# suryanshkumar/online-joint-depthfusion-and-semantic

Hardware: AMD Instinct MI355X
Metric: frames/sec fused (320x240, 256^3 grid) (higher is better)
Workload: dtype f16x3; 1 GPU; BASELINE configs[1]: 320x240 depth into a 256^3 fp16 TSDF grid, FusionNet_v3, geometry-only, fast integrate, f16x3 arithmetic, one scene per GPU; grid=256, n_points=9, n_tail_points=7, volume_dtype=f16, parallelism=scene-sharded x1, cpu_affinity=not pinned

## Files before the change

### include/ojf.h

```cpp
#ifndef OJF_H
#define OJF_H

#include <stddef.h>
#include <stdint.h>

#ifdef __cplusplus
extern "C" {
#endif

typedef void *ojf_stream_t;

#define OJF_MODE_FAST 0
#define OJF_MODE_PARITY 1

#define OJF_ACT_NONE 0
#define OJF_ACT_RELU 1
#define OJF_ACT_LEAKY 2
#define OJF_ACT_TANH 3

#define OJF_ARITH_F32 0
#define OJF_ARITH_F16X3 1

const char *ojf_version(void);
const char *ojf_last_error(void);
// ... 32 lines not shown
typedef struct ojf_net ojf_net;
typedef struct ojf_conv_layer {
    int c_in, c_out, ksize, dilation;
    const float *weight_host;
    const float *bias_host;
} ojf_conv_layer;

int ojf_net_create(ojf_net **out, int version, int n_points, int growth, int use_semantics,
                   float output_scale, const ojf_conv_layer *layers_host, int n_layers, int h,
                   int w);
void ojf_net_destroy(ojf_net *net);
int ojf_net_layer_count(int version, int n_points, int growth, int use_semantics);
int ojf_net_prepare_input(ojf_net *net, const float *values_dev, const float *weights_dev, int rows_stride,
                          int in_layout, const float *depth_dev, const uint8_t *sem_ids_dev, int n_classes,
                          ojf_stream_t stream);
int ojf_net_forward(ojf_net *net, float *est_dev, int est_stride, ojf_stream_t stream);
int64_t ojf_net_macs_per_pixel(const ojf_net *net);
int ojf_net_launch_count(const ojf_net *net);
int ojf_net_side_streams(ojf_net *net, ojf_stream_t stream, ojf_stream_t out[3]);
int ojf_net_profile(ojf_net *net, float *est_dev, int est_stride, ojf_stream_t stream, char *names, int names_cap,
                    float *micros, int max_entries);
int ojf_net_plan(int version, int n_points, int growth, int use_semantics, int h, int w, int arithmetic, char *names,
                 int names_cap);
int ojf_net_set_arithmetic(int arithmetic);
int ojf_net_get_arithmetic(const ojf_net *net);
int ojf_net_check(ojf_stream_t stream);
int ojf_guard_status(ojf_stream_t stream, int *flag, int *skipped);
int ojf_guard_poll(void);
int ojf_streams_overlap(ojf_stream_t a, ojf_stream_t b);

int ojf_conv2d(const float *in_dev, int in_stride, int in_off, float *out_dev, int out_stride,
               int out_off, const ojf_conv_layer *layer_host, int act, int h, int w,
               ojf_stream_t stream);

#define OJF_SEG_ACT_ZERO_PAD 0x100
typedef struct ojf_segconv ojf_segconv;
int ojf_segconv_create(ojf_segconv **out, const float *weight_host, const float *scale_host, const float *bias_host,
                       int c_in, int c_out, int ksize, int stride, int dilation, int padding);
int ojf_segdeconv_create(ojf_segconv **out, const float *weight_host, const float *scale_host, const float *bias_host,
                         int c_in, int c_out, int stride);
void ojf_segconv_destroy(ojf_segconv *conv);
int ojf_segconv_set_dropout(ojf_segconv *conv, const unsigned long long *rng_state_dev, unsigned stream_id, int advance);
int ojf_segconv_forward(const ojf_segconv *conv, const float *in_dev, int in_stride, float *out_dev, int out_stride,
                        const float *res_dev, int res_stride, const float *mul_dev, int mul_stride, int act, int h,
                        int w, ojf_stream_t stream);
int ojf_segconv_forward_group(int n, const ojf_segconv *const *convs, const float *const *ins_dev, int in_stride,
                              float *const *outs_dev, int out_stride, const float *const *ress_dev, int res_stride,
                              const float *const *muls_dev, int mul_stride, int act, int h, int w, ojf_stream_t stream);
int ojf_segconv_forward_multi(int n, int batch, const ojf_segconv *const *convs, const float *const *ins_dev, const int *in_strides,
                              float *const *outs_dev, const int *out_strides, const float *const *ress_dev, const int *res_strides,
                              const float *const *muls_dev, const int *mul_strides, const int *acts, const int *hs, const int *ws,
                              ojf_stream_t stream);
int ojf_segconv_forward_batch(const ojf_segconv *conv, int batch, const float *in_dev, int in_stride, float *out_dev, int out_stride,
                              const float *res_dev, int res_stride, const float *mul_dev, int mul_stride, int act, int h,
                              int w, ojf_stream_t stream);
int ojf_segconv_forward_group_batch(int n, int batch, const ojf_segconv *const *convs, const float *const *ins_dev, int in_stride,
                                    float *const *outs_dev, int out_stride, const float *const *ress_dev, int res_stride,
                                    const float *const *muls_dev, int mul_stride, int act, int h, int w, ojf_stream_t stream);

size_t ojf_train_packed_floats(int c_out_phys, int c_in_phys, int ksize);
int ojf_train_pack(const float *w_dev, const float *bias_dev, int oc, int ic, int ksize, int group, int slot, int c_in_phys,
                   int c_out_phys, int transposed, float *packed_dev, float *bias_packed_dev, ojf_stream_t stream);
int ojf_train_conv(const float *in_dev, int in_g0, int c_in_phys, float *out_dev, int out_g0, int c_out_phys,
                   const float *packed_dev, const float *bias_packed_dev, int ksize, int dilation, int h, int w, ojf_stream_t stream);
int ojf_train_avgpool3(const float *in_dev, float *out_dev, int c_phys, int h, int w, ojf_stream_t stream);
size_t ojf_train_partial_doubles(int c_phys);
// ... 201 lines not shown
```

### online_joint_depthfusion_and_semantic_amd/_lib.py

```python
import ctypes
import os

import numpy as np

_HERE = os.path.dirname(os.path.abspath(__file__))
LIB_PATH = os.path.join(_HERE, 'libojf.so')
if os.environ.get('OJF_LIB_PATH'):
    LIB_PATH = os.environ['OJF_LIB_PATH']

MODE_FAST = 0
MODE_PARITY = 1
ACT_NONE, ACT_RELU, ACT_LEAKY, ACT_TANH = 0, 1, 2, 3
ARITH_F32, ARITH_F16X3 = 0, 1
ARITHMETIC = {'f32': ARITH_F32, 'f16x3': ARITH_F16X3}


class OjfError(RuntimeError):
    pass


class ConvLayer(ctypes.Structure):
    _fields_ = [('c_in', ctypes.c_int), ('c_out', ctypes.c_int), ('ksize', ctypes.c_int),
                ('dilation', ctypes.c_int), ('weight_host', ctypes.c_void_p),
                ('bias_host', ctypes.c_void_p)]
# ... 35 lines not shown

SIGNATURES = {
    'ojf_version': (_c.c_char_p, []),
    'ojf_last_error': (_c.c_char_p, []),
    'ojf_device_count': (_i, []),
    'ojf_extract': (_i, [_vp, _vp, _vp, _vp, _d, _vp, _vp, _i, _i, _i, _i, _i, _i, _f, _vp, _vp, _i, _i,
                         _vp, _vp, _vp, _vp, _vp]),
    'ojf_extract_to_net': (_i, [_vp, _vp, _vp, _vp, _d, _vp, _vp, _i, _i, _i, _i, _i, _i, _f, _vp, _vp]),
    'ojf_extract_many': (_i, [_i, _c.POINTER(ExtractJob), _i, _i, _i, _i, _i, _i, _f, _vp]),
    'ojf_integrate_many': (_i, [_i, _c.POINTER(IntegrateJob), _i, _i, _f, _i, _i, _i, _i, _i, _vp]),
    'ojf_integrate_workspace_bytes': (_sz, [_i, _i, _i, _i, _i, _i, _i]),
    'ojf_integrate_workspace_init': (_i, [_vp, _sz, _i, _i, _i, _i, _i, _i, _i, _vp]),
    'ojf_integrate': (_i, [_vp, _vp, _vp, _vp, _d, _vp, _i, _i, _i, _f, _vp, _vp, _vp, _vp, _vp, _vp,
                           _i, _i, _i, _i, _i, _i, _vp, _sz, _vp, _vp]),
    'ojf_integrate_masked': (_i, [_vp, _vp, _vp, _vp, _vp, _d, _vp, _i, _i, _i, _f, _vp, _vp, _vp, _vp, _vp, _vp,
                                  _i, _i, _i, _i, _i, _i, _vp, _sz, _vp, _vp]),
    'ojf_integrate_entries': (_i, [_vp, _vp, _vp, _vp, _vp, _c.c_int64, _vp, _vp, _vp, _vp, _i, _i, _i, _vp, _sz, _vp, _vp]),
    'ojf_net_create': (_i, [_c.POINTER(_vp), _i, _i, _i, _i, _f, _c.POINTER(ConvLayer), _i, _i, _i]),
    'ojf_net_destroy': (None, [_vp]),
    'ojf_net_layer_count': (_i, [_i, _i, _i, _i]),
    'ojf_net_prepare_input': (_i, [_vp, _vp, _vp, _i, _i, _vp, _vp, _i, _vp]),
    'ojf_net_forward': (_i, [_vp, _vp, _i, _vp]),
    'ojf_net_macs_per_pixel': (_c.c_int64, [_vp]),
    'ojf_net_launch_count': (_i, [_vp]),
    'ojf_net_side_streams': (_i, [_vp, _vp, _vp]),
    'ojf_net_profile': (_i, [_vp, _vp, _i, _vp, _c.c_char_p, _i, _c.POINTER(_f), _i]),
    'ojf_net_plan': (_i, [_i, _i, _i, _i, _i, _i, _i, _c.c_char_p, _i]),
    'ojf_net_set_arithmetic': (_i, [_i]),
    'ojf_net_get_arithmetic': (_i, [_vp]),
    'ojf_net_check': (_i, [_vp]),
    'ojf_guard_status': (_i, [_vp, _c.POINTER(_i), _c.POINTER(_i)]),
    'ojf_guard_poll': (_i, []),
    'ojf_streams_overlap': (_i, [_vp, _vp]),
    'ojf_conv2d': (_i, [_vp, _i, _i, _vp, _i, _i, _c.POINTER(ConvLayer), _i, _i, _i, _vp]),
    'ojf_volume_fill_f16': (_i, [_vp, _sz, _f, _vp]),
    'ojf_volume_fill_u8': (_i, [_vp, _sz, _c.c_uint8, _vp]),
    'ojf_volume_filter': (_i, [_vp, _vp, _sz, _f, _f, _vp]),
    'ojf_volume_median5_u8': (_i, [_vp, _vp, _i, _i, _i, _vp]),
    'ojf_volume_evaluate': (_i, [_vp, _vp, _vp, _sz, _vp, _vp]),
    'ojf_volume_confusion': (_i, [_vp, _vp, _vp, _sz, _i, _vp, _vp, _vp]),
    'ojf_segconv_create': (_i, [_c.POINTER(_vp), _vp, _vp, _vp, _i, _i, _i, _i, _i, _i]),
    'ojf_segdeconv_create': (_i, [_c.POINTER(_vp), _vp, _vp, _vp, _i, _i, _i]),
    'ojf_segconv_destroy': (None, [_vp]),
    'ojf_segconv_forward': (_i, [_vp, _vp, _i, _vp, _i, _vp, _i, _vp, _i, _i, _i, _i, _vp]),
    'ojf_segconv_forward_batch': (_i, [_vp, _i, _vp, _i, _vp, _i, _vp, _i, _vp, _i, _i, _i, _i, _vp]),
    'ojf_segconv_forward_group': (_i, [_i, _vp, _vp, _i, _vp, _i, _vp, _i, _vp, _i, _i, _i, _i, _vp]),
    'ojf_segconv_forward_multi': (_i, [_i, _i, _vp, _vp, _vp, _vp, _vp, _vp, _vp, _vp, _vp, _vp, _vp, _vp, _vp]),
    'ojf_segconv_forward_group_batch': (_i, [_i, _i, _vp, _vp, _i, _vp, _i, _vp, _i, _vp, _i, _i, _i, _i, _vp]),
    'ojf_train_packed_floats': (_sz, [_i, _i, _i]),
    'ojf_train_pack': (_i, [_vp, _vp, _i, _i, _i, _i, _i, _i, _i, _i, _vp, _vp, _vp]),
    'ojf_train_conv': (_i, [_vp, _i, _i, _vp, _i, _i, _vp, _vp, _i, _i, _i, _i, _vp]),
    'ojf_train_avgpool3': (_i, [_vp, _vp, _i, _i, _i, _vp]),
    'ojf_train_partial_doubles': (_sz, [_i]),
    'ojf_train_channel_sums': (_i, [_vp, _i, _i, _i, _i, _vp, _vp]),
    'ojf_train_bn_act': (_i, [_vp, _i, _vp, _i, _i, _i, _i, _i, _vp, _vp, _vp, _i, _f, _i, _i, _f, _f, _vp, _vp, _vp, _vp, _vp, _vp]),
    'ojf_train_bn_act_bwd': (_i, [_vp, _i, _vp, _i, _vp, _i, _i, _i, _i, _i, _vp, _vp, _vp, _vp, _vp, _i, _f, _i, _i, _vp,
                                  _vp, _vp, _vp, _i, _vp]),
    'ojf_train_wgrad_partial_floats': (_sz, [_i, _i, _i, _i, _i]),
    'ojf_train_wgrad': (_i, [_vp, _i, _i, _vp, _i, _i, _i, _i, _i, _i, _i, _i, _i, _i, _vp, _vp, _i, _vp]),
    'ojf_trainer_create': (_i, [_c.POINTER(_vp), _i, _i, _i, _i, _f, _i, _i]),
    'ojf_trainer_destroy': (None, [_vp]),
    'ojf_trainer_set_arithmetic': (_i, [_vp, _i]),
    'ojf_trainer_set_backward_arithmetic': (_i, [_vp, _i]),
    'ojf_trainer_layer_count': (_i, [_vp]),
    'ojf_trainer_launch_count': (_i, [_vp]),
    'ojf_trainer_set_graph': (_i, [_vp, _i]),
# ... 123 lines not shown
```

### online_joint_depthfusion_and_semantic_amd/csrc/ojf_net.hip

```cpp
#include <chrono>
#include <cmath>
#include <cstdio>
#include <cstdlib>
#include <cstring>
#include <vector>

#include "ojf_common.h"

namespace ojf {

typedef float f32x4 __attribute__((ext_vector_type(4)));
typedef float f32x8 __attribute__((ext_vector_type(8)));
typedef _Float16 f16x8 __attribute__((ext_vector_type(8)));

typedef unsigned u32x4 __attribute__((ext_vector_type(4)));
__device__ __forceinline__ void split_f16(const f32x4 &a, const f32x4 &b, f16x8 &hi, f16x8 &lo)
{
    const f32x8 x = __builtin_shufflevector(a, b, 0, 1, 2, 3, 4, 5, 6, 7);
    hi = __builtin_convertvector(x, f16x8);
    const u32x4 h = __builtin_bit_cast(u32x4, hi);
    u32x4 l;
#pragma unroll
    for (int i = 0; i < 4; ++i) l[i] = split_lo_pair(h[i], x[2 * i], x[2 * i + 1]);
    lo = __builtin_bit_cast(f16x8, l);
// ... 899 lines not shown
    }
}

template <int ARITH, int MT, int NTIN, int NTOUT>
__device__ __forceinline__ void chain_run(f32x4 (&x)[MT][8], f32x4 (&y)[MT][8], f32x4 *wlds, const f32x4 *wg,
                                          const float *bias, const ChainArgs &a, const int (&p)[MT], int lane,
                                          f32x4 (&pre)[kChainPre], int &buf, VecStage &vs)
{
    chain_layer<ARITH, MT, NTIN, NTOUT, kChainLastRows, 0>(x, y, wlds, wg, a, p, lane, pre, buf, vs);
}

template <int ARITH, int MT, int NTIN, int NTOUT, int NTNEXT, int... REST>
__device__ __forceinline__ void chain_run(f32x4 (&x)[MT][8], f32x4 (&y)[MT][8], f32x4 *wlds, const f32x4 *wg,
                                          const float *bias, const ChainArgs &a, const int (&p)[MT], int lane,
                                          f32x4 (&pre)[kChainPre], int &buf, VecStage &vs)
{
    VecNext nx;
    nx.a = bias + chain_bias_stride(ARITH, NTOUT);
    nx.na = chain_bias_stride(ARITH, NTNEXT) / 4;
    chain_layer<ARITH, MT, NTIN, NTOUT, kChainLeaky, chain_first_size(ARITH, NTOUT, NTNEXT)>(x, y, wlds, wg, a, p, lane, pre,
                                                                                             buf, vs, nx);
    chain_run<ARITH, MT, NTOUT, NTNEXT, REST...>(y, x, wlds, wg + (size_t)chain_layer_size(ARITH, NTIN, NTOUT),
                                                 bias + chain_bias_stride(ARITH, NTOUT), a, p, lane, pre, buf, vs);
}

constexpr int kColShards = 16;
constexpr float kColScale = 1048576.0f;

constexpr int kColMax = 256;
struct ColSums {
    long long fix[kColShards][kColMax];
    unsigned bad[kColMax];
};
constexpr int colsum_row(int nt) { return nt > 8 ? 256 : 128; }

template <int MT, int NT, int NA>
__device__ __forceinline__ void block_colsum(const f32x4 (&x)[MT][NA], const int (&p)[MT], int npix, float *red ,
                                             ColSums *out, int lane, int wave, int off = 0)
{
    constexpr int RS = colsum_row(NT);
    const int g = lane >> 4;
#pragma unroll
    for (int S = 0; S < NT; ++S) {
        f32x4 s{0.f, 0.f, 0.f, 0.f};
#pragma unroll
        for (int m = 0; m < MT; ++m)
            if (p[m] < npix) s += x[m][S];
#pragma unroll
        for (int j = 0; j < 4; ++j) {
            float v = s[j];
            v += __shfl_xor(v, 8, 64);
            v += __shfl_xor(v, 4, 64);
            v += __shfl_xor(v, 2, 64);
            v += __shfl_xor(v, 1, 64);
            s[j] = v;
        }
        if ((lane & 15) == 0) *reinterpret_cast<f32x4 *>(red + wave * RS + S * 16 + 4 * g) = s;
    }
    __syncthreads();
    static_assert(NT * 16 <= kChainThreads && NT * 16 <= kColMax, "one thread per channel");
    if ((int)threadIdx.x < NT * 16) {
        const int t = threadIdx.x;
        float v = (red[t] + red[RS + t]) + (red[2 * RS + t] + red[3 * RS + t]);
#pragma unroll
        for (int w4 = 4; w4 < kChainWaves; w4 += 4)
            v += (red[w4 * RS + t] + red[(w4 + 1) * RS + t]) + (red[(w4 + 2) * RS + t] + red[(w4 + 3) * RS + t]);
// ... 183 lines not shown
        ca.out_planes = a.entry_out; ca.out_g0 = 0; ca.og_store = a.entry_og; ca.act_n = a.entry_act_n; ca.split_groups = a.entry_split;
        chain_layer<ARITH, MT, 8, 5, kChainEntry, 0>(y, t, wlds, a.entry_w, ca, p, lane, pre, buf, vs);
    } else if constexpr (CHAIN) {
        ca.out_rows = a.out_rows; ca.rows_stride = a.rows_stride; ca.rows_n = a.rows_n; ca.scale = a.scale;
        head_run<ARITH, MT, CHAIN>(y, t, wlds, a.chain_w, a.chain_b, ca, p, lane, pre, buf, vs);
    }
}

struct GaveArgs {
    const float *partial;
    struct ColSums *fixed;
    int nparts, pstride, cphys, npix;
    const float *WgT, *bg, *WfgT, *bf;
    int c_out;
    float *bias_out;
    int bias_len;
};

struct PyramidArgs {
    const f32x4 *z;
    f32x4 *q[3];
    const float *bias[3];
    int h, w, c4;
    int tiles;
    int fold_gave;
    const f32x4 *z2 = nullptr;
    f32x4 *q0 = nullptr;
    const float *bias0 = nullptr;
    int split_out;
    GaveArgs gave;
};

constexpr int kPoolTW = 32, kPoolTH = 8, kPoolStride = kPoolTW + 6;

template <int LV>
__device__ __forceinline__ void pool_pyramid_body(const PyramidArgs &a, f32x4 (&buf)[2][kPoolStride * (kPoolTH + 6)], int cg)
{
    const int tiles_x = (a.w + kPoolTW - 1) / kPoolTW;
    const int tile = banded_block_x();
    const int ty = tile / tiles_x, tx = tile - ty * tiles_x;
    const int x0 = tx * kPoolTW, y0 = ty * kPoolTH, npix = a.h * a.w;
    const f32x4 *plane = a.z + (size_t)(LV * a.c4 + cg) * npix;
    const f32x4 *plane2 = a.z2 ? a.z2 + (size_t)(LV * a.c4 + cg) * npix : nullptr;
    const f32x4 zero{0.f, 0.f, 0.f, 0.f};
    {
        constexpr int W0 = kPoolTW + 2 * LV, H0 = kPoolTH + 2 * LV;
#pragma unroll
        for (int i0 = 0; i0 < W0 * H0; i0 += 256) {
            const int i = i0 + threadIdx.x;
            if (i >= W0 * H0) break;
            const int ly = i / W0, lx = i - ly * W0;
            const int gy = y0 - LV + ly, gx = x0 - LV + lx;
            const bool in = (unsigned)gy < (unsigned)a.h && (unsigned)gx < (unsigned)a.w;
            f32x4 v = in ? plane[gy * a.w + gx] : zero;
            if (plane2 && in) v += plane2[gy * a.w + gx];
            buf[0][ly * kPoolStride + lx] = v;
        }
    }
    __syncthreads();
#pragma unroll
    for (int l = 1; l <= LV; ++l) {
        const int halo = LV - l;
        const int Wl = kPoolTW + 2 * halo, Hl = kPoolTH + 2 * halo;
        const f32x4 *src = buf[(l - 1) & 1];
#pragma unroll
        for (int i0 = 0; i0 < Wl * Hl; i0 += 256) {
            const int i = i0 + threadIdx.x;
            if (i >= Wl * Hl) break;
            const int ly = i / Wl, lx = i - ly * Wl;
            const int gy = y0 - halo + ly, gx = x0 - halo + lx;
            const bool in = (unsigned)gy < (unsigned)a.h && (unsigned)gx < (unsigned)a.w;
            f32x4 s = zero;
#pragma unroll
            for (int dy = 0; dy < 3; ++dy)
#pragma unroll
                for (int dx = 0; dx < 3; ++dx) s += src[(ly + dy) * kPoolStride + lx + dx];
            s = s / 9.0f;
            if (l < LV) {
                buf[l & 1][ly * kPoolStride + lx] = in ? s : zero;
            } else if (in) {
                s += *reinterpret_cast<const f32x4 *>(a.bias[LV - 1] + 4 * cg);
#pragma unroll
                for (int j = 0; j < 4; ++j) s[j] = s[j] < 0.0f ? 0.0f : s[j];
                a.q[LV - 1][(size_t)cg * npix + gy * a.w + gx] = a.split_out ? split_pack4(s) : s;
            }
        }
        if (l < LV) __syncthreads();
    }
}

__device__ __forceinline__ void gave_bias_block(const GaveArgs &a, float *mean, float *gv);

__global__ __launch_bounds__(256) void pool_pyramid_kernel(const PyramidArgs a)
{
    __shared__ f32x4 buf[2][kPoolStride * (kPoolTH + 6)];
    if (banded_block_x() >= a.tiles) {
        if (blockIdx.y == 0 && banded_block_x() == a.tiles && a.fold_gave)
            gave_bias_block(a.gave, reinterpret_cast<float *>(buf), reinterpret_cast<float *>(buf) + 256);
        return;
    }
    const int yg = blockIdx.y / a.c4, cg = blockIdx.y - yg * a.c4;
    const int lv = yg < 3 ? 3 - yg : 4;
    if (lv == 4) {
        const int tiles_x = (a.w + kPoolTW - 1) / kPoolTW;
        const int tile = banded_block_x();
        const int ty = tile / tiles_x, tx = tile - ty * tiles_x;
        const int gy = ty * kPoolTH + (int)threadIdx.x / kPoolTW, gx = tx * kPoolTW + (int)threadIdx.x % kPoolTW;
        if (gy < a.h && gx < a.w) {
            const size_t at = (size_t)cg * a.h * a.w + gy * a.w + gx;
            f32x4 v = a.z[at] + a.z2[at] + *reinterpret_cast<const f32x4 *>(a.bias0 + 4 * cg);
#pragma unroll
            for (int j = 0; j < 4; ++j) v[j] = v[j] < 0.0f ? 0.0f : v[j];
            a.q0[at] = a.split_out ? split_pack4(v) : v;
        }
        return;
    }
    if (lv == 1) pool_pyramid_body<1>(a, buf, cg);
    else if (lv == 2) pool_pyramid_body<2>(a, buf, cg);
    else pool_pyramid_body<3>(a, buf, cg);
}

constexpr int kSumBlocks = 32;

__global__ __launch_bounds__(256) void colsum_kernel(const f32x4 *in, int g0, int npix, float *partial)
{
    __shared__ f32x4 red[4];
    const int cg = blockIdx.y;
    const int per = (npix + gridDim.x - 1) / gridDim.x;
    const int p0 = blockIdx.x * per, p1 = min(npix, p0 + per);
    const f32x4 *plane = in + (size_t)(g0 + cg) * npix;
    f32x4 s{0.f, 0.f, 0.f, 0.f};
    for (int p = p0 + threadIdx.x; p < p1; p += 256) s += plane[p];
#pragma unroll
    for (int j = 0; j < 4; ++j)
        for (int off = 32; off > 0; off >>= 1) s[j] += __shfl_down(s[j], off, 64);
    if ((threadIdx.x & 63) == 0) red[threadIdx.x >> 6] = s;
    __syncthreads();
    if (threadIdx.x == 0) {
        s = (red[0] + red[1]) + (red[2] + red[3]);
        *reinterpret_cast<f32x4 *>(partial + (size_t)blockIdx.x * 256 + 4 * cg) = s;
    }
}


__device__ __forceinline__ void gave_bias_block(const GaveArgs &a, float *mean , float *gv )
{
    const int t = threadIdx.x;
    if (a.fixed) {
        if (t < kColMax) {
            long long q = 0;
#pragma unroll
            for (int sh = 0; sh < kColShards; ++sh) {
                q += a.fixed->fix[sh][t];
                a.fixed->fix[sh][t] = 0;
            }
            const bool bad = a.fixed->bad[t] != 0;
            a.fixed->bad[t] = 0;
            const float sum = (float)((double)q * (1.0 / (double)kColScale));
            mean[t] = t < a.cphys ? (bad ? __builtin_nanf("") : sum / (float)a.npix) : 0.0f;
        }
    } else if (a.cphys <= 128) {
        const int ch = t & 127, half = t >> 7;
        float s = 0.0f;
        if (ch < a.cphys) {
            const int r0 = half ? (a.nparts + 1) / 2 : 0, r1 = half ? a.nparts : (a.nparts + 1) / 2;
#pragma unroll 8
            for (int b = r0; b < r1; ++b) s += a.partial[(size_t)b * a.pstride + ch];
        }
        gv[t] = s;
        __syncthreads();
        mean[t] = t < a.cphys ? (gv[t] + gv[128 + t]) / (float)a.npix : 0.0f;
    } else {
        float s = 0.0f;
        if (t < a.cphys) {
#pragma unroll 8
            for (int b = 0; b < a.nparts; ++b) s += a.partial[(size_t)b * a.pstride + t];
        }
        mean[t] = s / (float)a.npix;
    }
    __syncthreads();
    float s1 = 0.0f;
    if (t < a.c_out) {
        s1 = a.bg[t];
#pragma unroll 8
        for (int c = 0; c < a.cphys; ++c) s1 = __builtin_fmaf(a.WgT[(size_t)c * a.c_out + t], mean[c], s1);
    }
    __syncthreads();
    gv[t] = s1;
    __syncthreads();
    if (t < a.bias_len) {
        float s = 0.0f;
        if (t < a.c_out) {
            s = a.bf[t];
#pragma unroll 8
            for (int j = 0; j < a.c_out; ++j) s = __builtin_fmaf(a.WfgT[(size_t)j * a.c_out + t], gv[j], s);
        }
        a.bias_out[t] = s;
    }
}

__global__ __launch_bounds__(256) void gave_bias_kernel(const GaveArgs a)
{
    __shared__ float mean[256];
    __shared__ float gv[256];
    gave_bias_block(a, mean, gv);
}

struct PrepArgs {
    const float *values;
    const float *weights;
    const float *depth;
    const uint8_t *sem;
    f32x4 *x0;
    f32x4 *x1;
    int rows_stride, in_layout, npix, P, cs4, n_classes, v2_sem;
    int *ovf;
    int split;
};

__global__ __launch_bounds__(256) void prepare_input_kernel(const PrepArgs a)
{
    const int p = blockIdx.x * blockDim.x + threadIdx.x;
    if (p >= a.npix) return;
    const size_t pix = a.in_layout ? (size_t)p : (size_t)p * a.rows_stride;
    const size_t chn = a.in_layout ? (size_t)a.rows_stride : 1;
    const float *v = a.values + pix;
    const float *wt = a.weights + pix;
    const float d = a.depth[p];
    const float sf = a.sem ? (1.0f + (float)a.sem[p]) / (float)a.n_classes : 0.0f;
    bool bad = false;
    for (int cg = 0; cg < a.cs4; ++cg) {
        f32x4 r0, r1;
#pragma unroll
        for (int j = 0; j < 4; ++j) {
            const int c = 4 * cg + j;
            float base = 0.0f;
            if (c < a.P) base = v[c * chn];
            else if (c < 2 * a.P) base = wt[(c - a.P) * chn];
// ... 938 lines not shown
            if (upload(ew, &v.entry_w) || upload(eb, &v.entry_b)) return -2;
            if (half_entry_form(c_in_phys, cs, os)) {
                const std::vector<float> zero_bias(4 * cs, 0.0f);
                for (int hd = 0; hd < 2; ++hd) {
                    auto wh = [&](int oc, int k) { return oc < 4 * cs && k < net->os ? b.W[(size_t)oc * c_in_phys + hd * net->os + k] : 0.0f; };
                    const std::vector<float> rh = chain_row_scales(net->arith, 5, net->os, wh);
                    std::vector<float> hw, hb;
                    pack_chain_layer(hw, net->arith, 5, 8, rh, wh);
                    append_chain_bias(hb, net->arith, 5, 4 * cs, zero_bias.data(), rh);
                    if (upload(hw, &v.entry_wh[hd]) || upload(hb, &v.entry_bh[hd])) return -2;
                }
                std::vector<float> b0(cs, 0.0f);
                for (int o = 0; o < cs; ++o) b0[o] = b.B[o];
                if (upload(b0, &v.bias0)) return -2;
            }
        }
    }
    const std::vector<int> id_c = slot_map(c, c, cs);
    for (int br = 0; br < 4; ++br) {
        const ojf_conv_layer &la = L[2 + 4 * br], &lb = L[3 + 4 * br], &l1 = L[4 + 4 * br];
        if (la.c_in != c || la.c_out != c || lb.c_in != c || lb.c_out != c || l1.c_in != c || l1.c_out != out)
            return fail("ojf_net_create: branch conv shape mismatch");
        ConvBuilder ba(cs, cs, 3, la.dilation), bb(cs, cs, 3, lb.dilation), b1(cs, os, 1, 1);
        ba.add(la, 0, c, id_c, 0, true);
        bb.add(lb, 0, c, id_c, 0, true);
        b1.add(l1, 0, c, id_c, 0, true);
        if (finish(ba, v.b3a[br], net->arith) || finish(bb, v.b3b[br], net->arith) || finish(b1, v.b1[br], net->arith)) return -2;
    }
    {
        const ojf_conv_layer &lf = L[17];
        ConvBuilder b(4 * os, os, 1, 1);
        b.add(lf, out, 5 * out, slot_map(4 * out, out, os), 0, false);
        if (finish(b, v.fin, net->arith)) return -2;
        std::vector<float> Wg((size_t)out * c_in_phys, 0.0f), bg(out), Wfg((size_t)out * out), bf(out);
        for (int o = 0; o < out; ++o) {
            for (int ci = 0; ci < c_in; ++ci) Wg[(size_t)in_map[ci] * out + o] = L[0].weight_host[(size_t)o * c_in + ci];
            bg[o] = L[0].bias_host[o];
            for (int j = 0; j < out; ++j) Wfg[(size_t)j * out + o] = lf.weight_host[(size_t)o * 5 * out + j];
            bf[o] = lf.bias_host[o];
        }
        if (upload(Wg, &v.Wg) || upload(bg, &v.bg) || upload(Wfg, &v.Wfg) || upload(bf, &v.bf)) return -2;
        std::vector<float> zero((size_t)v.fin.n_ot * 16, 0.0f);
        if (upload(zero, &v.bias_final)) return -2;
    }
    if (fused_tail_form(cs, os)) {
        const int NV = 2, NO = 8;
        std::vector<float> tw, tb;
        const ojf_conv_layer &lf = L[17];
        const std::vector<float> rf = chain_row_scales(net->arith, NO, 4 * out, [&](int oc, int k) {
            return oc < out ? lf.weight_host[(size_t)oc * 5 * out + out + k] : 0.0f;
        });
        for (int br = 0; br < 4; ++br) {
            const ojf_conv_layer &l1 = L[4 + 4 * br];
            auto w1 = [&](int oc, int k) { return oc < out && k < c ? l1.weight_host[(size_t)oc * c + k] : 0.0f; };
            const std::vector<float> r1 = chain_row_scales(net->arith, NO, c, w1);
            pack_chain_layer(tw, net->arith, NO, NV, r1, w1);
            pack_chain_layer(tw, net->arith, NO, NO, rf, [&](int oc, int k) {
                return oc < out && k < out ? lf.weight_host[(size_t)oc * 5 * out + out * (br + 1) + k] : 0.0f;
            });
            append_chain_bias(tb, net->arith, NO, out, l1.bias_host, r1);
        }
        std::vector<float> rfi(rf.size());
        for (size_t i = 0; i < rf.size(); ++i) rfi[i] = 1.0f / rf[i];
        if (upload(rfi, &v.tail_rinv)) return -2;
        if (upload(tw, &v.tail_w) || upload(tb, &v.tail_b1)) return -2;
    }
    return 0;
}

static void free_vortex(Vortex &v)
{
    release(v.stacked);
    release(v.fin);
    for (int b = 0; b < 4; ++b) {
        release(v.b3a[b]);
        release(v.b3b[b]);
        release(v.b1[b]);
        if (v.pool_bias[b]) (void)hipFree(v.pool_bias[b]);
    }
    float *ptrs[] = {v.Wg, v.bg, v.Wfg, v.bf, v.bias_final, v.tail_w, v.tail_b1, v.tail_rinv, v.entry_w, v.entry_b,
                     v.entry_wh[0], v.entry_wh[1], v.entry_bh[0], v.entry_bh[1], v.bias0};
    for (float *p : ptrs)
        if (p) (void)hipFree(p);
}

static GaveArgs gave_args(const ojf_net *net, const Vortex &v, const float *partial, int nparts, int pstride, ColSums *fixed = nullptr)
{
    GaveArgs ga;
    ga.partial = partial; ga.fixed = fixed; ga.nparts = nparts; ga.pstride = pstride; ga.cphys = v.c_in_phys; ga.npix = net->npix;
    ga.WgT = v.Wg; ga.bg = v.bg; ga.WfgT = v.Wfg; ga.bf = v.bf; ga.c_out = net->pool_in;
    ga.bias_out = v.bias_final; ga.bias_len = v.fin.n_ot * 16;
    return ga;
}

static int chain_blocks(const ojf_net *net) { return ((net->npix + 15) / 16 + ojf::kChainWaves - 1) / ojf::kChainWaves; }

#define OJF_LAUNCH_BY_ARITH(KERNEL, ARGS, ...)                                                                              \
    do {                                                                                                                     \
        if (h16) hipLaunchKernelGGL((KERNEL<OJF_ARITH_F16X3, __VA_ARGS__>), grid, block, 0, st, ARGS);                      \
        else hipLaunchKernelGGL((KERNEL<OJF_ARITH_F32, __VA_ARGS__>), grid, block, 0, st, ARGS);                            \
    } while (0)

static int run_vortex(ojf_net *net, const VortexStep &s, hipStream_t st, const ChainArgs &head)
{
    const int h = net->h, w = net->w, c4 = net->cs / 4, o4 = net->os / 4;
    const bool h16 = net->arith == OJF_ARITH_F16X3;
    const bool last = s.vortex == 2;
    const Vortex &v = net->vortex[s.vortex], &next = net->vortex[2];
    ojf_net::Scratch &sc = net->sc[s.set];
    const float *in = last ? net->YY : net->X[s.vortex];
    float *out = last ? net->Y3 : net->YY;
    const int in_g0 = 0, out_g0 = last ? 0 : s.vortex * o4;
    const dim3 grid(chain_blocks(net)), block(ojf::kChainThreads);
    const int banded = (grid.x & 7) == 0 ? 1 : 0;

    if (s.entry == ENTRY_GENERIC) {
        OJF_HIP(hipEventRecord(sc.ev_fork, st));
        OJF_HIP(hipStreamWaitEvent(sc.side, sc.ev_fork, 0));
        const dim3 sgrid(kSumBlocks, v.c_in_phys / 4), ggrid(1);
        hipLaunchKernelGGL(colsum_kernel, sgrid, dim3(256), 0, sc.side, planes(in), in_g0, net->npix, sc.partial);
        if (net_trace_on()) fprintf(stderr, "ojf_net %s | grid_x %u grid_y %u\n", kLaunchNames[L_COLSUM], sgrid.x, sgrid.y);
        mark_launch(L_COLSUM, sc.side);
        OJF_HIP(hipGetLastError());
        hipLaunchKernelGGL(gave_bias_kernel, ggrid, dim3(256), 0, sc.side, gave_args(net, v, sc.partial, kSumBlocks, 256));
        if (net_trace_on()) fprintf(stderr, "ojf_net %s | grid_x %u grid_y %u\n", kLaunchNames[L_GAVE_BIAS], ggrid.x, ggrid.y);
        mark_launch(L_GAVE_BIAS, sc.side);
        OJF_HIP(hipGetLastError());
        if (launch_conv(v.stacked, in, in_g0, sc.Z, 0, nullptr, OJF_ACT_RELU, net->cs, 1.0f, h, w, st)) return -2;
        OJF_HIP(hipEventRecord(sc.ev_entry, st));
    } else if (s.entry == ENTRY_KERNEL) {
        ChainArgs ea;
        ea.in = planes(in); ea.w = planes(v.entry_w); ea.bias = v.entry_b; ea.out_rows = nullptr;
        ea.in_g0 = in_g0; ea.c4_in = v.c_in_phys / 4; ea.npix = net->npix; ea.rows_stride = 0; ea.rows_n = 0; ea.scale = 1.0f;
        ea.ovf = h16 ? overflow_flag() : nullptr;
        ea.out_planes = planes(sc.Z); ea.out_g0 = 0; ea.og_store = 4 * c4; ea.act_n = net->cs; ea.colsum = sc.colsum;
        ea.split_groups = s.split ? c4 : 0;
        ea.in_split = s.in_split ? 1 : 0;
        if (s.entry_ntin == 16) OJF_LAUNCH_BY_ARITH(entry1x1_kernel, ea, 1, 16, 5);
        else OJF_LAUNCH_BY_ARITH(entry1x1_kernel, ea, 1, 8, 5);
        if (net_trace_on())
            fprintf(stderr, "ojf_net %s | ntin %d blocks %u banded %d\n", kLaunchNames[L_ENTRY1X1], s.entry_ntin, grid.x, banded);
        mark_launch(L_ENTRY1X1, st);
        OJF_HIP(hipGetLastError());
    }

    {
        PyramidArgs pa;
        pa.z = planes(sc.Z);
        pa.q[0] = planes(sc.Q1); pa.q[1] = planes(sc.Q2); pa.q[2] = planes(sc.Q3);
        for (int b = 0; b < 3; ++b) pa.bias[b] = v.pool_bias[b + 1];
        pa.h = h; pa.w = w; pa.c4 = c4;
        pa.tiles = ((w + kPoolTW - 1) / kPoolTW) * ((h + kPoolTH - 1) / kPoolTH);
        pa.gave = gave_args(net, v, nullptr, 0, 0, s.z2 ? net->colsum3 : sc.colsum);
        pa.fold_gave = s.chain_flow ? 1 : 0;
        pa.split_out = s.split ? 1 : 0;
        if (s.z2) { pa.z2 = planes(net->sc[1].Z); pa.q0 = planes(sc.Q0); pa.bias0 = v.bias0; }
        const dim3 pgrid(round_up(pa.tiles + (s.chain_flow ? 1 : 0), 8), (s.z2 ? 4 : 3) * c4);
        hipLaunchKernelGGL(pool_pyramid_kernel, pgrid, dim3(256), 0, st, pa);
        if (net_trace_on()) fprintf(stderr, "ojf_net %s | tiles %d grid_x %u grid_y %u\n", kLaunchNames[L_POOL_PYRAMID], pa.tiles, pgrid.x, pgrid.y);
        mark_launch(L_POOL_PYRAMID, st);
        OJF_HIP(hipGetLastError());
    }
    const float *bin[4] = {s.z2 ? sc.Q0 : sc.Z, sc.Q1, sc.Q2, sc.Q3};
    {
        ConvArgs ga[4], gb[4];
        for (int br = 0; br < 4; ++br) {
            fill_conv_args(ga[br], v.b3a[br], bin[br], 0, sc.U, br * c4, nullptr, OJF_ACT_RELU, net->cs, 1.0f, h, w);
            fill_conv_args(gb[br], v.b3b[br], sc.U, br * c4, sc.V, br * c4, nullptr, OJF_ACT_RELU, net->cs, 1.0f, h, w);
            ga[br].in_split = ga[br].out_split = gb[br].in_split = s.split ? 1 : 0;
        }
        if (s.branches == BRANCH_GROUPED) {
            if (launch_conv_args(ga, 4, v.b3a[0].n_ot, st, net->arith)) return -2;
            if (launch_conv_args(gb, 4, v.b3b[0].n_ot, st, net->arith)) return -2;
        } else {
            OJF_HIP(hipStreamWaitEvent(sc.side, sc.ev_entry, 0));
            if (launch_conv_args(ga, 1, v.b3a[0].n_ot, sc.side, net->arith)) return -2;
            if (launch_conv_args(gb, 1, v.b3b[0].n_ot, sc.side, net->arith)) return -2;
            if (launch_conv_args(ga + 1, 3, v.b3a[1].n_ot, st, net->arith)) return -2;
            if (launch_conv_args(gb + 1, 3, v.b3b[1].n_ot, st, net->arith)) return -2;
        }
    }

    if (!s.chain_flow) {
        OJF_HIP(hipEventRecord(sc.ev_join, sc.side));
        OJF_HIP(hipStreamWaitEvent(st, sc.ev_join, 0));
    }
    if (s.tail == TAIL_UNFUSED) {
        for (int br = 0; br < 4; ++br)
            if (launch_conv(v.b1[br], sc.V, br * c4, sc.CAT, br * o4, nullptr, OJF_ACT_RELU, net->os, 1.0f, h, w, st))
                return -2;
        return launch_conv(v.fin, sc.CAT, 0, out, out_g0, v.bias_final, OJF_ACT_NONE, 0, 1.0f, h, w, st);
// ... 599 lines not shown
{
    using namespace ojf;
    if (!in || !out || !layer || !layer->weight_host || !layer->bias_host) return fail("ojf_conv2d: null pointer argument");
    if ((layer->ksize != 1 && layer->ksize != 3) || layer->dilation < 1) return fail("ojf_conv2d: 1x1 or 3x3 kernels only");
    const int cin_phys = round_up(layer->c_in, 4), cout_phys = round_up(layer->c_out, 4);
    if (in_off + layer->c_in > in_stride || out_off + cout_phys > out_stride)
        return fail("ojf_conv2d: channel window exceeds the row stride");
    hipStream_t st = as_stream(stream);
    const int npix = h * w;
    ConvBuilder b(cin_phys, cout_phys, layer->ksize, layer->dilation);
    b.add(*layer, 0, layer->c_in, slot_map(layer->c_in, layer->c_in, cin_phys), 0, true);
    PackedConv pc;
    if (finish(b, pc, g_default_arith)) return -2;
    float *pin = nullptr, *pout = nullptr;
    int rc = alloc_planes(&pin, npix, cin_phys);
    if (!rc) rc = alloc_planes(&pout, npix, cout_phys);
    if (!rc) {
        hipLaunchKernelGGL(rows_to_planes_kernel, dim3((npix * (cin_phys / 4) + 255) / 256), dim3(256), 0, st, in, in_stride,
                           in_off, layer->c_in, planes(pin), cin_phys / 4, npix);
        rc = launch_conv(pc, pin, 0, pout, 0, nullptr, act, cout_phys, 1.0f, h, w, st);
    }
    if (!rc) {
        hipLaunchKernelGGL(planes_to_rows_kernel, dim3((npix * (cout_phys / 4) + 255) / 256), dim3(256), 0, st,
                           planes(pout), cout_phys / 4, npix, out, out_stride, out_off);
        rc = check_hip(hipStreamSynchronize(st), "ojf_conv2d sync");
        if (!rc && guard_take(nullptr, true)) rc = fail(kOverflowMsg);
    }
    free_planes(pin);
    free_planes(pout);
    release(pc);
    return rc;
}

#include "ojf_net_train.h"
#include "ojf_train_net.h"
```

Measured before the change: 2713 frames/sec.

## Restructure pool pyramid: batched loads, row-pair pooling, prefetched gave-bias fold

The pool pyramid now issues all of its tile loads before any LDS store, and each thread computes two output rows from shared 3-wide row reads. A reciprocal-multiply div9 with a correction step replaces the per-element divide. The gave-bias fold block now streams its weight matrices through LDS in double-buffered register chunks, so each thread no longer reads weights serially and global latency is hidden. The column-sum shard reduction is split across all 256 threads. This also adds a standalone ojf_pool_pyramid API and optional timestamp instrumentation, and pads the weight buffers to a multiple of four for vector loads.

```diff
diff --git a/include/ojf.h b/include/ojf.h
--- a/include/ojf.h
+++ b/include/ojf.h
@@ -88,6 +88,12 @@
 int ojf_conv2d(const float *in_dev, int in_stride, int in_off, float *out_dev, int out_stride,
                int out_off, const ojf_conv_layer *layer_host, int act, int h, int w,
                ojf_stream_t stream);
+
+int ojf_pool_pyramid(const float *z_dev, const float *z2_dev, float *q1_dev, float *q2_dev, float *q3_dev, float *q0_dev,
+                     const float *bias1_dev, const float *bias2_dev, const float *bias3_dev, const float *bias0_dev, int h, int w,
+                     int c4, int split_out, void *colsums_dev, const float *wg_t_dev, const float *bg_dev,
+                     const float *wfg_t_dev, const float *bf_dev, int cphys, int c_out, float *bias_out_dev, int bias_len,
+                     ojf_stream_t stream);
 
 #define OJF_SEG_ACT_ZERO_PAD 0x100
 typedef struct ojf_segconv ojf_segconv;
diff --git a/online_joint_depthfusion_and_semantic_amd/_lib.py b/online_joint_depthfusion_and_semantic_amd/_lib.py
--- a/online_joint_depthfusion_and_semantic_amd/_lib.py
+++ b/online_joint_depthfusion_and_semantic_amd/_lib.py
@@ -91,6 +91,7 @@
     'ojf_guard_status': (_i, [_vp, _c.POINTER(_i), _c.POINTER(_i)]),
     'ojf_guard_poll': (_i, []),
     'ojf_streams_overlap': (_i, [_vp, _vp]),
+    'ojf_pool_pyramid': (_i, [_vp] * 10 + [_i] * 4 + [_vp] * 5 + [_i, _i, _vp, _i, _vp]),
     'ojf_conv2d': (_i, [_vp, _i, _i, _vp, _i, _i, _c.POINTER(ConvLayer), _i, _i, _i, _vp]),
     'ojf_volume_fill_f16': (_i, [_vp, _sz, _f, _vp]),
     'ojf_volume_fill_u8': (_i, [_vp, _sz, _c.c_uint8, _vp]),
diff --git a/online_joint_depthfusion_and_semantic_amd/csrc/ojf_net.hip b/online_joint_depthfusion_and_semantic_amd/csrc/ojf_net.hip
--- a/online_joint_depthfusion_and_semantic_amd/csrc/ojf_net.hip
+++ b/online_joint_depthfusion_and_semantic_amd/csrc/ojf_net.hip
@@ -955,6 +955,7 @@
     long long fix[kColShards][kColMax];
     unsigned bad[kColMax];
 };
+static_assert(sizeof(ColSums) == kColShards * kColMax * 8 + kColMax * 4, "the layout include/ojf.h gives for ojf_pool_pyramid");
 constexpr int colsum_row(int nt) { return nt > 8 ? 256 : 128; }
 
 template <int MT, int NT, int NA>
@@ -1204,6 +1205,16 @@
 };
 
 constexpr int kPoolTW = 32, kPoolTH = 8, kPoolStride = kPoolTW + 6;
+constexpr int kPoolPH = 2;
+static_assert((kPoolTW + 4) * ((kPoolTH + 4 + kPoolPH - 1) / kPoolPH) <= 256, "one pass of the block covers the widest level");
+
+__device__ __forceinline__ float div9(float x)
+{
+    const float r = 1.0f / 9.0f;
+    const float q = x * r;
+    const float f = __builtin_fmaf(__builtin_fmaf(-9.0f, q, x), r, q);
+    return q == x ? x : f;
+}
 
 template <int LV>
 __device__ __forceinline__ void pool_pyramid_body(const PyramidArgs &a, f32x4 (&buf)[2][kPoolStride * (kPoolTH + 6)], int cg)
@@ -1216,59 +1227,98 @@
     const f32x4 *plane2 = a.z2 ? a.z2 + (size_t)(LV * a.c4 + cg) * npix : nullptr;
     const f32x4 zero{0.f, 0.f, 0.f, 0.f};
     {
-        constexpr int W0 = kPoolTW + 2 * LV, H0 = kPoolTH + 2 * LV;
-#pragma unroll
-        for (int i0 = 0; i0 < W0 * H0; i0 += 256) {
-            const int i = i0 + threadIdx.x;
-            if (i >= W0 * H0) break;
+        constexpr int W0 = kPoolTW + 2 * LV, H0 = kPoolTH + 2 * LV, N0 = (W0 * H0 + 255) / 256;
+        f32x4 v[N0];
+        int at[N0];
+#pragma unroll
+        for (int k = 0; k < N0; ++k) {
+            const int i = k * 256 + threadIdx.x;
             const int ly = i / W0, lx = i - ly * W0;
             const int gy = y0 - LV + ly, gx = x0 - LV + lx;
-            const bool in = (unsigned)gy < (unsigned)a.h && (unsigned)gx < (unsigned)a.w;
-            f32x4 v = in ? plane[gy * a.w + gx] : zero;
-            if (plane2 && in) v += plane2[gy * a.w + gx];
-            buf[0][ly * kPoolStride + lx] = v;
+            const bool in = i < W0 * H0 && (unsigned)gy < (unsigned)a.h && (unsigned)gx < (unsigned)a.w;
+            at[k] = in ? gy * a.w + gx : -1;
+            v[k] = in ? plane[at[k]] : zero;
+        }
+        if (plane2) {
+#pragma unroll
+            for (int k = 0; k < N0; ++k)
+                if (at[k] >= 0) v[k] += plane2[at[k]];
+        }
+#pragma unroll
+        for (int k = 0; k < N0; ++k) {
+            const int i = k * 256 + threadIdx.x;
+            const int ly = i / W0, lx = i - ly * W0;
+            if (i < W0 * H0) buf[0][ly * kPoolStride + lx] = v[k];
         }
     }
     __syncthreads();
 #pragma unroll
     for (int l = 1; l <= LV; ++l) {
         const int halo = LV - l;
-        const int Wl = kPoolTW + 2 * halo, Hl = kPoolTH + 2 * halo;
+        const int Wl = kPoolTW + 2 * halo, Hl = kPoolTH + 2 * halo, NP = (Hl + kPoolPH - 1) / kPoolPH;
+        const bool whole = Hl % kPoolPH == 0;
         const f32x4 *src = buf[(l - 1) & 1];
-#pragma unroll
-        for (int i0 = 0; i0 < Wl * Hl; i0 += 256) {
-            const int i = i0 + threadIdx.x;
-            if (i >= Wl * Hl) break;
-            const int ly = i / Wl, lx = i - ly * Wl;
-            const int gy = y0 - halo + ly, gx = x0 - halo + lx;
-            const bool in = (unsigned)gy < (unsigned)a.h && (unsigned)gx < (unsigned)a.w;
-            f32x4 s = zero;
-#pragma unroll
-            for (int dy = 0; dy < 3; ++dy)
-#pragma unroll
-                for (int dx = 0; dx < 3; ++dx) s += src[(ly + dy) * kPoolStride + lx + dx];
-            s = s / 9.0f;
-            if (l < LV) {
-                buf[l & 1][ly * kPoolStride + lx] = in ? s : zero;
-            } else if (in) {
-                s += *reinterpret_cast<const f32x4 *>(a.bias[LV - 1] + 4 * cg);
-#pragma unroll
-                for (int j = 0; j < 4; ++j) s[j] = s[j] < 0.0f ? 0.0f : s[j];
-                a.q[LV - 1][(size_t)cg * npix + gy * a.w + gx] = a.split_out ? split_pack4(s) : s;
+        const int i = threadIdx.x;
+        if (i < Wl * NP) {
+            const int pr = i / Wl, lx = i - pr * Wl, ly0 = pr * kPoolPH;
+            f32x4 acc[kPoolPH];
+#pragma unroll
+            for (int o = 0; o < kPoolPH; ++o) acc[o] = zero;
+#pragma unroll
+            for (int r = 0; r < kPoolPH + 2; ++r) {
+                if (whole || ly0 + r < Hl + 2) {
+                    const f32x4 *row = src + (ly0 + r) * kPoolStride + lx;
+                    const f32x4 t0 = row[0], t1 = row[1], t2 = row[2];
+#pragma unroll
+                    for (int o = 0; o < kPoolPH; ++o)
+                        if (r - o >= 0 && r - o <= 2) {
+                            acc[o] += t0;
+                            acc[o] += t1;
+                            acc[o] += t2;
+                        }
+                }
             }
+            const int gx = x0 - halo + lx;
+#pragma unroll
+            for (int o = 0; o < kPoolPH; ++o) {
+                const int ly = ly0 + o, gy = y0 - halo + ly;
+                if (!whole && ly >= Hl) break;
+                const bool in = (unsigned)gy < (unsigned)a.h && (unsigned)gx < (unsigned)a.w;
+                f32x4 s;
+#pragma unroll
+                for (int j = 0; j < 4; ++j) s[j] = div9(acc[o][j]);
+                if (l < LV) {
+                    buf[l & 1][ly * kPoolStride + lx] = in ? s : zero;
+                } else if (in) {
+                    s += *reinterpret_cast<const f32x4 *>(a.bias[LV - 1] + 4 * cg);
+#pragma unroll
+                    for (int j = 0; j < 4; ++j) s[j] = s[j] < 0.0f ? 0.0f : s[j];
+                    a.q[LV - 1][(size_t)cg * npix + gy * a.w + gx] = a.split_out ? split_pack4(s) : s;
+                }
+            }
         }
         if (l < LV) __syncthreads();
     }
 }
 
-__device__ __forceinline__ void gave_bias_block(const GaveArgs &a, float *mean, float *gv);
-
-__global__ __launch_bounds__(256) void pool_pyramid_kernel(const PyramidArgs a)
-{
-    __shared__ f32x4 buf[2][kPoolStride * (kPoolTH + 6)];
+constexpr int kGaveLds = 128 + 256 * 3;
+__device__ __forceinline__ void gave_bias_block(const GaveArgs &a, float *lds);
+
+#ifdef OJF_POOL_STAMPS
+constexpr int kPoolStampBlocks = 8192;
+__device__ unsigned long long g_pool_stamps[kPoolStampBlocks][2];
+#define POOL_STAMP(i) do { const unsigned b_ = blockIdx.y * gridDim.x + blockIdx.x; if (threadIdx.x == 0 && b_ < (unsigned)kPoolStampBlocks - 8) g_pool_stamps[b_][i] = wall_clock64(); } while (0)
+#define FOLD_STAMP(i) do { if (threadIdx.x == 0) g_pool_stamps[kPoolStampBlocks - 8 + (i)][0] = wall_clock64(); } while (0)
+#else
+#define POOL_STAMP(i) do { } while (0)
+#define FOLD_STAMP(i) do { } while (0)
+#endif
+
+__device__ __forceinline__ void pool_pyramid_block(const PyramidArgs &a, f32x4 (&buf)[2][kPoolStride * (kPoolTH + 6)])
+{
+    static_assert(2 * kPoolStride * (kPoolTH + 6) >= kGaveLds, "the fold block works in the pools' LDS");
     if (banded_block_x() >= a.tiles) {
-        if (blockIdx.y == 0 && banded_block_x() == a.tiles && a.fold_gave)
-            gave_bias_block(a.gave, reinterpret_cast<float *>(buf), reinterpret_cast<float *>(buf) + 256);
+        if (blockIdx.y == 0 && banded_block_x() == a.tiles && a.fold_gave) gave_bias_block(a.gave, reinterpret_cast<float *>(buf));
         return;
     }
     const int yg = blockIdx.y / a.c4, cg = blockIdx.y - yg * a.c4;
@@ -1292,6 +1342,14 @@
     else pool_pyramid_body<3>(a, buf, cg);
 }
 
+__global__ __launch_bounds__(256) void pool_pyramid_kernel(const PyramidArgs a)
+{
+    __shared__ f32x4 buf[2][kPoolStride * (kPoolTH + 6)];
+    POOL_STAMP(0);
+    pool_pyramid_block(a, buf);
+    POOL_STAMP(1);
+}
+
 constexpr int kSumBlocks = 32;
 
 __global__ __launch_bounds__(256) void colsum_kernel(const f32x4 *in, int g0, int npix, float *partial)
@@ -1315,22 +1373,99 @@
 }
 
 
-__device__ __forceinline__ void gave_bias_block(const GaveArgs &a, float *mean , float *gv )
+constexpr int kGavePer = 3, kGaveChunk = 256 * kGavePer;
+static_assert(kGaveLds == 128 + kGaveChunk, "float4: mean[256], gv[256], the chunk");
+
+struct GaveStream {
+    const float *W[2];
+    int rows[2];
+    int chunks[2];
+    int c_out, R;
+};
+
+__device__ __forceinline__ void gave_fetch(const GaveStream &gs, int g, f32x4 (&r)[kGavePer])
+{
+    g = min(g, gs.chunks[0] + gs.chunks[1] - 1);
+    const int m = g < gs.chunks[0] ? 0 : 1, k = m ? g - gs.chunks[0] : g;
+    const int f0 = k * gs.R * gs.c_out, last = (gs.rows[m] * gs.c_out - 1) & ~3;
+    const float *W = gs.W[m];
+#pragma unroll
+    for (int i = 0; i < kGavePer; ++i) r[i] = *reinterpret_cast<const f32x4 *>(W + min(f0 + 4 * (i * 256 + (int)threadIdx.x), last));
+}
+
+__device__ __forceinline__ void gave_step(const GaveArgs &a, const GaveStream &gs, int g, f32x4 (&r)[kGavePer], f32x4 *stage,
+                                          const float *mean, float *gv, float &s, float bf)
 {
     const int t = threadIdx.x;
+    if (g >= gs.chunks[0] + gs.chunks[1]) return;
+    const int m = g < gs.chunks[0] ? 0 : 1, k = m ? g - gs.chunks[0] : g;
+    __syncthreads();
+#pragma unroll
+    for (int i = 0; i < kGavePer; ++i) stage[i * 256 + t] = r[i];
+    if (m == 1 && k == 0) {
+        gv[t] = t < a.c_out ? s : 0.0f;
+        s = bf;
+        FOLD_STAMP(2);
+    }
+    gave_fetch(gs, g + 2, r);
+    __syncthreads();
+    if (t < a.c_out) {
+        const int n = min(gs.R, gs.rows[m] - k * gs.R);
+        const float *x = (m ? gv : mean) + k * gs.R, *wl = reinterpret_cast<const float *>(stage) + t;
+#pragma unroll 8
+        for (int c = 0; c < n; ++c) s = __builtin_fmaf(wl[c * a.c_out], x[c], s);
+    }
+}
+
+__device__ __forceinline__ void gave_bias_block(const GaveArgs &a, float *lds )
+{
+    float *mean = lds, *gv = lds + 256;
+    f32x4 *stage = reinterpret_cast<f32x4 *>(lds + 512);
+    const int t = threadIdx.x;
+    GaveStream gs;
+    gs.W[0] = a.WgT; gs.W[1] = a.WfgT;
+    gs.rows[0] = a.cphys; gs.rows[1] = a.c_out;
+    gs.c_out = a.c_out; gs.R = (4 * kGaveChunk / a.c_out) & ~3;
+    for (int m = 0; m < 2; ++m) gs.chunks[m] = (gs.rows[m] + gs.R - 1) / gs.R;
+    FOLD_STAMP(0);
+    f32x4 r0[kGavePer], r1[kGavePer];
+    gave_fetch(gs, 0, r0);
+    gave_fetch(gs, 1, r1);
+    const float bg = t < a.c_out ? a.bg[t] : 0.0f, bf = t < a.c_out ? a.bf[t] : 0.0f;
     if (a.fixed) {
-        if (t < kColMax) {
-            long long q = 0;
-#pragma unroll
-            for (int sh = 0; sh < kColShards; ++sh) {
-                q += a.fixed->fix[sh][t];
-                a.fixed->fix[sh][t] = 0;
+        long long *qs = reinterpret_cast<long long *>(stage);
+        static_assert(kColMax == 256, "one thread per channel");
+        const bool bad = a.fixed->bad[t] != 0;
+        a.fixed->bad[t] = 0;
+        long long q = 0;
+        if (a.cphys <= 128) {
+            const int ch = t & 127, s0 = (t >> 7) * 8;
+            long long part[8];
+#pragma unroll
+            for (int sh = 0; sh < 8; ++sh) part[sh] = a.fixed->fix[s0 + sh][ch];
+#pragma unroll
+            for (int sh = 0; sh < 8; ++sh) {
+                q += part[sh];
+                a.fixed->fix[s0 + sh][ch] = 0;
             }
-            const bool bad = a.fixed->bad[t] != 0;
-            a.fixed->bad[t] = 0;
-            const float sum = (float)((double)q * (1.0 / (double)kColScale));
-            mean[t] = t < a.cphys ? (bad ? __builtin_nanf("") : sum / (float)a.npix) : 0.0f;
-        }
+            if (t >= 128) qs[ch] = q;
+            __syncthreads();
+            if (t < 128) q += qs[t];
+        } else {
+#pragma unroll 1
+            for (int s0 = 0; s0 < kColShards; s0 += 8) {
+                long long part[8];
+#pragma unroll
+                for (int sh = 0; sh < 8; ++sh) part[sh] = a.fixed->fix[s0 + sh][t];
+#pragma unroll
+                for (int sh = 0; sh < 8; ++sh) {
+                    q += part[sh];
+                    a.fixed->fix[s0 + sh][t] = 0;
+                }
+            }
+        }
+        const float sum = (float)((double)q * (1.0 / (double)kColScale));
+        mean[t] = t < a.cphys ? (bad ? __builtin_nanf("") : sum / (float)a.npix) : 0.0f;
     } else if (a.cphys <= 128) {
         const int ch = t & 127, half = t >> 7;
         float s = 0.0f;
@@ -1350,32 +1485,21 @@
         }
         mean[t] = s / (float)a.npix;
     }
-    __syncthreads();
-    float s1 = 0.0f;
-    if (t < a.c_out) {
-        s1 = a.bg[t];
-#pragma unroll 8
-        for (int c = 0; c < a.cphys; ++c) s1 = __builtin_fmaf(a.WgT[(size_t)c * a.c_out + t], mean[c], s1);
-    }
-    __syncthreads();
-    gv[t] = s1;
-    __syncthreads();
-    if (t < a.bias_len) {
-        float s = 0.0f;
-        if (t < a.c_out) {
-            s = a.bf[t];
-#pragma unroll 8
-            for (int j = 0; j < a.c_out; ++j) s = __builtin_fmaf(a.WfgT[(size_t)j * a.c_out + t], gv[j], s);
-        }
-        a.bias_out[t] = s;
-    }
+    FOLD_STAMP(1);
+    float s = bg;
+    const int total = gs.chunks[0] + gs.chunks[1];
+    for (int g = 0; g < total; g += 2) {
+        gave_step(a, gs, g, r0, stage, mean, gv, s, bf);
+        gave_step(a, gs, g + 1, r1, stage, mean, gv, s, bf);
+    }
+    if (t < a.bias_len) a.bias_out[t] = t < a.c_out ? s : 0.0f;
+    FOLD_STAMP(3);
 }
 
 __global__ __launch_bounds__(256) void gave_bias_kernel(const GaveArgs a)
 {
-    __shared__ float mean[256];
-    __shared__ float gv[256];
-    gave_bias_block(a, mean, gv);
+    __shared__ f32x4 lds[kGaveLds];
+    gave_bias_block(a, reinterpret_cast<float *>(lds));
 }
 
 struct PrepArgs {
@@ -2380,7 +2504,7 @@
         ConvBuilder b(4 * os, os, 1, 1);
         b.add(lf, out, 5 * out, slot_map(4 * out, out, os), 0, false);
         if (finish(b, v.fin, net->arith)) return -2;
-        std::vector<float> Wg((size_t)out * c_in_phys, 0.0f), bg(out), Wfg((size_t)out * out), bf(out);
+        std::vector<float> Wg(((size_t)out * c_in_phys + 3) / 4 * 4, 0.0f), bg(out), Wfg(((size_t)out * out + 3) / 4 * 4, 0.0f), bf(out);
         for (int o = 0; o < out; ++o) {
             for (int ci = 0; ci < c_in; ++ci) Wg[(size_t)in_map[ci] * out + o] = L[0].weight_host[(size_t)o * c_in + ci];
             bg[o] = L[0].bias_host[o];
@@ -2439,6 +2563,14 @@
     ga.WgT = v.Wg; ga.bg = v.bg; ga.WfgT = v.Wfg; ga.bf = v.bf; ga.c_out = net->pool_in;
     ga.bias_out = v.bias_final; ga.bias_len = v.fin.n_ot * 16;
     return ga;
+}
+
+static dim3 launch_pyramid(PyramidArgs &pa, hipStream_t st)
+{
+    pa.tiles = ((pa.w + kPoolTW - 1) / kPoolTW) * ((pa.h + kPoolTH - 1) / kPoolTH);
+    const dim3 pgrid(round_up(pa.tiles + (pa.fold_gave ? 1 : 0), 8), (pa.z2 ? 4 : 3) * pa.c4);
+    hipLaunchKernelGGL(pool_pyramid_kernel, pgrid, dim3(256), 0, st, pa);
+    return pgrid;
 }
 
 static int chain_blocks(const ojf_net *net) { return ((net->npix + 15) / 16 + ojf::kChainWaves - 1) / ojf::kChainWaves; }
@@ -2498,13 +2630,11 @@
         pa.q[0] = planes(sc.Q1); pa.q[1] = planes(sc.Q2); pa.q[2] = planes(sc.Q3);
         for (int b = 0; b < 3; ++b) pa.bias[b] = v.pool_bias[b + 1];
         pa.h = h; pa.w = w; pa.c4 = c4;
-        pa.tiles = ((w + kPoolTW - 1) / kPoolTW) * ((h + kPoolTH - 1) / kPoolTH);
         pa.gave = gave_args(net, v, nullptr, 0, 0, s.z2 ? net->colsum3 : sc.colsum);
         pa.fold_gave = s.chain_flow ? 1 : 0;
         pa.split_out = s.split ? 1 : 0;
         if (s.z2) { pa.z2 = planes(net->sc[1].Z); pa.q0 = planes(sc.Q0); pa.bias0 = v.bias0; }
-        const dim3 pgrid(round_up(pa.tiles + (s.chain_flow ? 1 : 0), 8), (s.z2 ? 4 : 3) * c4);
-        hipLaunchKernelGGL(pool_pyramid_kernel, pgrid, dim3(256), 0, st, pa);
+        const dim3 pgrid = launch_pyramid(pa, st);
         if (net_trace_on()) fprintf(stderr, "ojf_net %s | tiles %d grid_x %u grid_y %u\n", kLaunchNames[L_POOL_PYRAMID], pa.tiles, pgrid.x, pgrid.y);
         mark_launch(L_POOL_PYRAMID, st);
         OJF_HIP(hipGetLastError());
@@ -3170,5 +3300,42 @@
     return rc;
 }
 
+OJF_API int ojf_pool_pyramid(const float *z, const float *z2, float *q1, float *q2, float *q3, float *q0, const float *bias1,
+                             const float *bias2, const float *bias3, const float *bias0, int h, int w, int c4, int split_out,
+                             void *colsums, const float *wg_t, const float *bg, const float *wfg_t, const float *bf, int cphys,
+                             int c_out, float *bias_out, int bias_len, ojf_stream_t stream)
+{
+    using namespace ojf;
+    if (!z || !q1 || !q2 || !q3 || !bias1 || !bias2 || !bias3) return fail("ojf_pool_pyramid: null pointer argument");
+    if (z2 && (!q0 || !bias0)) return fail("ojf_pool_pyramid: z2 needs q0 and bias0");
+    if (h < 1 || w < 1 || c4 < 1 || c4 > 64 || (int64_t)h * w > (1 << 24)) return fail("ojf_pool_pyramid: bad frame size or group count");
+    PyramidArgs pa;
+    pa.z = planes(z); pa.z2 = z2 ? planes(z2) : nullptr;
+    pa.q[0] = planes(q1); pa.q[1] = planes(q2); pa.q[2] = planes(q3); pa.q0 = z2 ? planes(q0) : nullptr;
+    pa.bias[0] = bias1; pa.bias[1] = bias2; pa.bias[2] = bias3; pa.bias0 = z2 ? bias0 : nullptr;
+    pa.h = h; pa.w = w; pa.c4 = c4;
+    pa.split_out = split_out ? 1 : 0;
+    pa.fold_gave = colsums ? 1 : 0;
+    pa.gave = GaveArgs{};
+    if (colsums) {
+        if (!wg_t || !bg || !wfg_t || !bf || !bias_out) return fail("ojf_pool_pyramid: null pointer argument (fold)");
+        if (cphys < 1 || cphys > kColMax || c_out < 1 || c_out > 256 || bias_len < 0 || bias_len > 256)
+            return fail("ojf_pool_pyramid: fold sizes beyond one block (256)");
+        GaveArgs &ga = pa.gave;
+        ga.partial = nullptr; ga.fixed = static_cast<ColSums *>(colsums); ga.nparts = 0; ga.pstride = 0; ga.cphys = cphys; ga.npix = h * w;
+        ga.WgT = wg_t; ga.bg = bg; ga.WfgT = wfg_t; ga.bf = bf; ga.c_out = c_out;
+        ga.bias_out = bias_out; ga.bias_len = bias_len;
+    }
+    launch_pyramid(pa, as_stream(stream));
+    return check_hip(hipGetLastError(), "ojf_pool_pyramid launch");
+}
+
+#ifdef OJF_POOL_STAMPS
+extern "C" __attribute__((visibility("default"))) int ojf_debug_pool_stamps(void *host_dst, size_t bytes)
+{
+    return (int)hipMemcpyFromSymbol(host_dst, HIP_SYMBOL(ojf::g_pool_stamps), bytes < sizeof(ojf::g_pool_stamps) ? bytes : sizeof(ojf::g_pool_stamps));
+}
+#endif
+
 #include "ojf_net_train.h"
 #include "ojf_train_net.h"
```

After: 2757 frames/sec (median of 6 runs). +1.6%, better.
